# mli43/Cuda-Optimization-for-SpMM

Hardware: AMD Instinct MI355X
Metric: SpMM GFLOP/s, large_25605 (n4c6-b13) CSR x dense K=128 fp32 (higher is better)
Workload: dtype f32

## Files before the change

cuda-optimization-for-spmm_amd/csrc/row_gather.hpp:

```cpp
#pragma once
#include <algorithm>
#include <cstdio>
#include <cstdlib>
#include <type_traits>

#include "spmm_common.hpp"

namespace mispmm {

#ifdef MISPMM_STAMPS
static __device__ unsigned long long *mispmm_stamp_buf = nullptr;
constexpr uint32_t kStampLaunches = 32;
#endif

struct CsrRows {
    const uint32_t *rowPtrs;
    static constexpr bool kPadded = false;
    __device__ __forceinline__ void extent(uint32_t row, size_t &base, uint32_t &len) const {
        const uint32_t s = rowPtrs[row];
        base = s;
        len = rowPtrs[row + 1] - s;
    }
};

struct UniformRows {
    uint32_t width;
    static constexpr bool kPadded = false;
    __device__ __forceinline__ void extent(uint32_t row, size_t &base, uint32_t &len) const {
        base = static_cast<size_t>(row) * width;
        len = width;
    }
};

struct EllRows {
    uint32_t width;
    static constexpr bool kPadded = true;
    __device__ __forceinline__ void extent(uint32_t row, size_t &base, uint32_t &len) const {
        base = static_cast<size_t>(row) * width;
        len = width;
    }
};

struct SpanRows {
    const uint32_t *spans;
    static constexpr bool kPadded = false;
};

constexpr uint32_t kMaxBatch = 16;
struct BatchPtrs {
    const float *b[kMaxBatch];
    float *c[kMaxBatch];
};
template <bool BATCHED> struct BatchArg {};
template <> struct BatchArg<true> {
    BatchPtrs p;
};

template <int G, int VEC, class Acc, bool CBUF, class Rows, int BLOCK = 256, int UMAX = 16, bool ROLL = false, int SLOTS = 16,
          bool BATCHED = false, bool MAPPED = false>
#ifndef MISPMM_X_WAVES
#define MISPMM_X_WAVES 5
#endif
__device__ __forceinline__ void row_gather_body(const uint32_t bx, const uint32_t by, const uint32_t bz,
    uint32_t M, uint32_t rb_chunk, uint32_t tiling, uint32_t cols_per_part, uint32_t N, uint32_t ldb, Rows rows,
    const uint32_t *__restrict__ colIdxs, const float *__restrict__ vals, uint32_t b_bytes,
    const float *__restrict__ B_one, float *__restrict__ C_one, uint32_t c_bytes, uint32_t ldc,
    const uint32_t *__restrict__ rowMap, BatchArg<BATCHED> batch
#ifdef MISPMM_STAMPS
    , uint32_t stamp_launch
#endif
    ) {
#ifdef MISPMM_STAMPS
    unsigned long long stamp[5];
    stamp[0] = wall_clock64();
#endif
#ifdef MISPMM_X_PRIO
    __builtin_amdgcn_s_setprio(3);
#endif
    const float *__restrict__ B = B_one;
    float *__restrict__ C = C_one;
    if constexpr (BATCHED) {
        B = batch.p.b[bz];
        C = batch.p.c[bz];
    }
    constexpr int GROUPS = BLOCK / G;
    constexpr int U = G < UMAX ? G : UMAX;
    using vec_t = typename VecOf<VEC>::type;
    const uint32_t lane = threadIdx.x % G;
    const uint32_t xcd = bx & 7u, slot = bx >> 3;
    const uint32_t log2p = tiling & 0xFFu;
    const uint32_t p = xcd & ((1u << log2p) - 1u), q = xcd >> log2p;
    const uint32_t row = (p * rb_chunk + slot) * GROUPS + threadIdx.x / G;
    const bool row_ok = row < M;
    const uint32_t col0 = q * cols_per_part + by * (G * VEC) + lane * VEC;
    const bool col_ok = col0 < min(N, (q + 1) * cols_per_part);
    size_t row_base = 0;
    uint32_t row_len = 0;
    uint32_t ptr_lo = 0, ptr_hi = 0;
    uint32_t out_row = row;
    if constexpr (std::is_same_v<Rows, CsrRows>) {
        const uint32_t rr = min(row, M - 1u);
        ptr_lo = rows.rowPtrs[rr];
        ptr_hi = rows.rowPtrs[rr + 1];
    } else if constexpr (std::is_same_v<Rows, SpanRows>) {
        if (row_ok) {
            using u4 = uint32_t __attribute__((ext_vector_type(4)));
            const u4 span = *reinterpret_cast<const u4 *>(rows.spans + static_cast<size_t>(row) * 4u);
            out_row = span[0];
            row_base = span[1];
            row_len = span[2] - span[1];
        }
    } else {
        if (row_ok) rows.extent(row, row_base, row_len);
    }
    auto resolve_extent = [&] {
        if constexpr (std::is_same_v<Rows, CsrRows>) {
            row_base = ptr_lo;
            row_len = row_ok ? ptr_hi - ptr_lo : 0u;
        }
    };
    typename Acc::T acc[VEC];
#pragma unroll
    for (int v = 0; v < VEC; ++v) acc[v] = 0;
    auto load_out_row = [&] {
        if constexpr (MAPPED) {
            if (row_ok) out_row = rowMap[row];
        }
    };
    const rsrc_t rsrc = make_rsrc(B, b_bytes);
    const uint32_t lane_off = col_ok ? col0 * 4u : kDropLoad;
    const uint32_t ldb4 = ldb * 4u;

    auto fetch = [&](size_t mine, uint32_t &off, float &val) {
        const uint32_t col = colIdxs[mine];
        val = vals[mine];
        off = col * ldb4;
        if constexpr (Rows::kPadded) {
            if (col == 0xFFFFFFFFu) {
                off = kDropLoad;
                val = 0.f;
            }
        }
    };
    auto issue = [&](auto nb_tag, vec_t *bv, float *av, uint32_t my_off, float my_val, uint32_t j, uint32_t cnt) {
        constexpr int NB = decltype(nb_tag)::value;
#pragma unroll
        for (int u = 0; u < NB; ++u) {
            const uint32_t src = (j + u) & (G - 1);
            const uint32_t off = __shfl(my_off, src, G);
            const float a = __shfl(my_val, src, G);
            bool live = j + u < cnt;
            if constexpr (Rows::kPadded) live = live && off != kDropLoad;
            av[u] = live ? a : 0.f;
            bv[u] = buffer_load_vec<VEC>(rsrc, live ? off + lane_off : kDropLoad, 0);
        }
    };
    auto consume = [&](auto nb_tag, const vec_t *bv, const float *av) {
        constexpr int NB = decltype(nb_tag)::value;
#pragma unroll
        for (int u = 0; u < NB; ++u) {
#pragma unroll
            for (int v = 0; v < VEC; ++v) Acc::mac(acc[v], av[u], vec_get<VEC>(bv[u], v));
        }
    };
    using FullBatch = std::integral_constant<int, U>;

    if constexpr (ROLL && G <= 16) {
        constexpr int SC = SLOTS, E = (SC + G - 1) / G;
        static_assert(SLOTS == 16 || (SLOTS > U && SLOTS < 16) || (G == 16 && SLOTS == 32), "unsupported slot count");
        uint32_t nxt_off[E];
        float nxt_val[E];
        auto fetch_super = [&](uint32_t base) {
#pragma unroll
            for (int e = 0; e < E; ++e) {
                const uint32_t idx = base + e * G + lane;
                fetch(row_base + min(idx, row_len - 1), nxt_off[e], nxt_val[e]);
                if (idx >= row_len) {
                    nxt_off[e] = kDropLoad;
                    nxt_val[e] = 0.f;
                }
            }
        };
        if constexpr (std::is_same_v<Rows, CsrRows>) {
            const uint32_t guess = tiling >> 8;
            if (guess != 0) {
                row_base = static_cast<size_t>(row) * guess;
                row_len = row_ok ? guess : 0u;
                if (row_len != 0) fetch_super(0);
                const size_t bet_base = row_base;
                const uint32_t bet_len = row_len;
                resolve_extent();
                const bool hit = __all(!row_ok || (row_base == bet_base && row_len == bet_len));
                if (!hit && row_len != 0) fetch_super(0);
            } else {
                resolve_extent();
                if (row_len != 0) fetch_super(0);
            }
        } else {
            if (row_len != 0) fetch_super(0);
        }
        load_out_row();
#ifdef MISPMM_X_PRIO
        __builtin_amdgcn_s_setprio(0);
#endif
#ifdef MISPMM_STAMPS
        asm volatile("s_waitcnt vmcnt(0)" ::: "memory");
        stamp[1] = wall_clock64();
#endif
        for (uint32_t base = 0; base < row_len; base += SC) {
            uint32_t my_off[E];
            float my_val[E];
#pragma unroll
            for (int e = 0; e < E; ++e) {
                my_off[e] = nxt_off[e];
                my_val[e] = nxt_val[e];
            }
            if (base + SC < row_len) fetch_super(base + SC);
            vec_t bv[U];
            float av[U];
            auto issue_one = [&](auto slot_tag, vec_t &b, float &a) {
                constexpr int S = decltype(slot_tag)::value;
                const uint32_t off = group_bcast<G, S % G>(my_off[S / G]);
                const float c = __builtin_bit_cast(float, group_bcast<G, S % G>(__builtin_bit_cast(uint32_t, my_val[S / G])));
                a = c;
                b = buffer_load_vec<VEC, MISPMM_B_LOAD_AUX>(rsrc, off + lane_off, 0);
            };
            auto consume_one = [&](const vec_t &b, float a) {
                if constexpr (VEC == 4 && std::is_same_v<Acc, AccRefWide>) {
                    Acc::mac4(acc, a, vec_get<VEC>(b, 0), vec_get<VEC>(b, 1), vec_get<VEC>(b, 2), vec_get<VEC>(b, 3));
                } else {
#pragma unroll
                    for (int v = 0; v < VEC; ++v) Acc::mac(acc[v], a, vec_get<VEC>(b, v));
                }
            };
            auto live_from = [&](auto from_tag) {
                constexpr int FROM = decltype(from_tag)::value;
                bool live = false;
                static_for<0, E>([&](auto e_tag) {
                    constexpr int E0 = decltype(e_tag)::value * G;
                    if constexpr (E0 + G > FROM) {
                        const bool in_range = (E0 >= FROM) || (lane >= static_cast<uint32_t>(FROM > E0 ? FROM - E0 : 0));
                        live = live || (in_range && my_off[decltype(e_tag)::value] != kDropLoad);
                    }
                });
                return __any(live);
            };
            auto roll = [&](auto scx_tag) {
                constexpr int SCX = decltype(scx_tag)::value;
                static_for<0, U>([&](auto s) { issue_one(s, bv[decltype(s)::value], av[decltype(s)::value]); });
                __builtin_amdgcn_sched_barrier(0);
                static_for<0, SCX>([&](auto s) {
                    constexpr int S = decltype(s)::value;
                    consume_one(bv[S % U], av[S % U]);
                    if constexpr (S + U < SCX) {
                        if constexpr (VEC == 4) asm volatile("" : "+v"(acc[0]), "+v"(acc[1]), "+v"(acc[2]), "+v"(acc[3]) : : "memory");
                        else if constexpr (VEC == 2) asm volatile("" : "+v"(acc[0]), "+v"(acc[1]) : : "memory");
                        else asm volatile("" : "+v"(acc[0]) : : "memory");
                        __builtin_amdgcn_sched_barrier(0);
                        issue_one(std::integral_constant<int, S + U>{}, bv[S % U], av[S % U]);
                        __builtin_amdgcn_sched_barrier(0);
                    }
                });
            };
            if constexpr (Rows::kPadded) {
                if (!live_from(std::integral_constant<int, 0>{})) continue;
            }
            if (!live_from(std::integral_constant<int, U>{})) {
                static_for<0, U>([&](auto s) { issue_one(s, bv[decltype(s)::value], av[decltype(s)::value]); });
                __builtin_amdgcn_sched_barrier(0);
                static_for<0, U>([&](auto s) { consume_one(bv[decltype(s)::value], av[decltype(s)::value]); });
            } else if constexpr (SC == 16) {
#ifdef MISPMM_X_FEWBODIES
                if (!live_from(std::integral_constant<int, 14>{})) roll(std::integral_constant<int, 14>{});
                else roll(std::integral_constant<int, 16>{});
#else
                if (!live_from(std::integral_constant<int, 10>{})) roll(std::integral_constant<int, 10>{});
                else if (!live_from(std::integral_constant<int, 12>{})) roll(std::integral_constant<int, 12>{});
                else if (!live_from(std::integral_constant<int, 14>{})) roll(std::integral_constant<int, 14>{});
                else roll(std::integral_constant<int, 16>{});
#endif
            } else {
                roll(std::integral_constant<int, SC>{});
            }
        }
    } else if (resolve_extent(), !__any(row_len > static_cast<uint32_t>(U))) {
        load_out_row();
        if (row_len != 0) {
            uint32_t my_off;
            float my_val;
            fetch(row_base + min(lane, row_len - 1), my_off, my_val);
            vec_t bv[U];
            float av[U];
            issue(FullBatch{}, bv, av, my_off, my_val, 0, row_len);
            __builtin_amdgcn_sched_barrier(0);
            consume(FullBatch{}, bv, av);
        }
    } else {
        uint32_t nxt_off = 0;
        float nxt_val = 0.f;
        if (row_len != 0) fetch(row_base + min(lane, row_len - 1), nxt_off, nxt_val);
        load_out_row();
        for (uint32_t base = 0; base < row_len; base += G) {
            const uint32_t cnt = min(static_cast<uint32_t>(G), row_len - base);
            const uint32_t my_off = nxt_off;
            const float my_val = nxt_val;
            if (base + G < row_len) fetch(row_base + min(base + G + lane, row_len - 1), nxt_off, nxt_val);
            for (uint32_t j = 0; j < cnt; j += U) {
                vec_t bv[U];
                float av[U];
                issue(FullBatch{}, bv, av, my_off, my_val, j, cnt);
                __builtin_amdgcn_sched_barrier(0);
                consume(FullBatch{}, bv, av);
            }
        }
    }
#ifdef MISPMM_STAMPS
    if constexpr (VEC == 4) asm volatile("" : "+v"(acc[0]), "+v"(acc[1]), "+v"(acc[2]), "+v"(acc[3]) : : "memory");
    stamp[2] = wall_clock64();
#endif
    if (row_ok && col_ok) {
        vec_t out;
#pragma unroll
        for (int v = 0; v < VEC; ++v) vec_set<VEC>(out, v, Acc::finish(acc[v]));
        if constexpr (CBUF) {
            buffer_store_vec_c<VEC>(make_rsrc(C, c_bytes), (out_row * ldc + col0) * 4u, out);
        } else {
            store_vec<VEC>(C + static_cast<size_t>(out_row) * ldc + col0, out);
        }
    }
#ifdef MISPMM_STAMPS
    stamp[3] = wall_clock64();
    asm volatile("s_waitcnt vmcnt(0)" ::: "memory");
    stamp[4] = wall_clock64();
    if (mispmm_stamp_buf && (threadIdx.x & 63) == 0) {
        const uint32_t wpb = blockDim.x / 64;
        const size_t waves_per_launch = static_cast<size_t>(gridDim.x) * gridDim.y * wpb;
        unsigned long long *o = mispmm_stamp_buf + (stamp_launch * waves_per_launch +
            (static_cast<size_t>(by) * gridDim.x + bx) * wpb + (threadIdx.x >> 6)) * 8;
#pragma unroll
        for (int i = 0; i < 5; ++i) o[i] = stamp[i];
        o[5] = static_cast<unsigned long long>(__builtin_amdgcn_s_getreg((31 << 11) | 4));
        o[6] = static_cast<unsigned long long>(__builtin_amdgcn_s_getreg((31 << 11) | 20));
    }
#endif
}

template <int G, int VEC, class Acc, bool CBUF, class Rows, int BLOCK = 256, int UMAX = 16, bool ROLL = false, int SLOTS = 16,
          bool BATCHED = false, bool MAPPED = false>
__global__ __launch_bounds__(BLOCK, ROLL ? (UMAX > 8 ? 3 : MISPMM_X_WAVES) : 1) void row_gather_kernel(
    uint32_t M, uint32_t rb_chunk, uint32_t tiling, uint32_t cols_per_part, uint32_t N, uint32_t ldb, Rows rows,
    const uint32_t *__restrict__ colIdxs, const float *__restrict__ vals, uint32_t b_bytes,
    const float *__restrict__ B_one, float *__restrict__ C_one, uint32_t c_bytes, uint32_t ldc,
    const uint32_t *__restrict__ rowMap, BatchArg<BATCHED> batch
#ifdef MISPMM_STAMPS
    , uint32_t stamp_launch
#endif
    ) {
    row_gather_body<G, VEC, Acc, CBUF, Rows, BLOCK, UMAX, ROLL, SLOTS, BATCHED, MAPPED>(blockIdx.x, blockIdx.y, blockIdx.z, M, rb_chunk, tiling,
                                                                                    cols_per_part, N, ldb, rows, colIdxs, vals, b_bytes, B_one,
                                                                                    C_one, c_bytes, ldc, rowMap, batch
#ifdef MISPMM_STAMPS
                                                                                    , stamp_launch
#endif
    );
}

struct alignas(16) LineTail {
    float *C;
    uint32_t c_bytes, ldc4;
    const uint32_t *rowMap;
    uint64_t reserved;
};
struct LineBatchPair {
    const float *b;
    float *c;
};
template <bool BATCHED> struct LineBatch {};
template <> struct alignas(16) LineBatch<true> {
    LineBatchPair p[kMaxBatch];
};

template <int G, class Acc, bool PADDED, int SLOTS, bool BATCHED, bool MAPPED>
__global__ __launch_bounds__(128, MISPMM_X_WAVES) void row_line_kernel(
    const uint32_t *__restrict__ colIdxs, const float *__restrict__ vals, const float *__restrict__ B_one, uint32_t b_bytes,
    uint32_t ldb4, uint32_t width, uint32_t M, uint32_t rb_chunk, uint32_t log2p, uint32_t cols_per_part,
    LineTail tail, LineBatch<BATCHED> batch
#ifdef MISPMM_STAMPS
    , uint32_t stamp_launch
#endif
    ) {
#ifdef MISPMM_STAMPS
    unsigned long long stamp[5];
    stamp[0] = wall_clock64();
#endif
    constexpr int VEC = 4, BLOCK = 128, GROUPS = BLOCK / G, U = 8, E = (SLOTS + G - 1) / G;
    static_assert((G == 8 || G == 16) && SLOTS > U && SLOTS < 16, "rows of 9..14 slots");
    using vec_t = f32x4;
    const float *__restrict__ B = B_one;
    float *__restrict__ C = tail.C;
    const uint32_t c_bytes = tail.c_bytes, ldc4 = tail.ldc4;
    const uint32_t *__restrict__ rowMap = tail.rowMap;
    if constexpr (BATCHED) {
        const LineBatchPair pr = batch.p[blockIdx.z];
        B = pr.b;
        C = pr.c;
    }
    __builtin_amdgcn_sched_barrier(0);
    const uint32_t lane = threadIdx.x % G;
    const uint32_t xcd = blockIdx.x & 7u, slot = blockIdx.x >> 3;
    const uint32_t p = xcd & ((1u << log2p) - 1u), q = xcd >> log2p;
    const uint32_t row = (p * rb_chunk + slot) * GROUPS + threadIdx.x / G;
    const bool row_ok = row < M;
    const uint32_t part_col = blockIdx.y * (G * VEC) + lane * VEC;
    const bool col_ok = part_col < cols_per_part;
    const uint32_t col0 = q * cols_per_part + part_col;

    const uint32_t a_bytes = M * width * 4u;
    const rsrc_t colrs = make_rsrc(colIdxs, a_bytes), valrs = make_rsrc(vals, a_bytes);
    const uint32_t row_pos = row * width;
    uint32_t raw_col[E], raw_val[E];
#pragma unroll
    for (int e = 0; e < E; ++e) {
        const uint32_t idx = static_cast<uint32_t>(e * G) + lane;
        const uint32_t pos4 = row_ok ? (row_pos + min(idx, width - 1u)) * 4u : kDropLoad;
        raw_col[e] = __builtin_amdgcn_raw_buffer_load_b32(colrs, pos4, 0, 0);
        raw_val[e] = __builtin_amdgcn_raw_buffer_load_b32(valrs, pos4, 0, 0);
    }
    __builtin_amdgcn_sched_barrier(0);
    uint32_t out_row = row;
    if constexpr (MAPPED) out_row = __builtin_amdgcn_raw_buffer_load_b32(make_rsrc(rowMap, M * 4u), row_ok ? row * 4u : kDropLoad, 0, 0);
    const rsrc_t brs = make_rsrc(B, b_bytes);
    const rsrc_t crs = make_rsrc(C, c_bytes);
    const uint32_t lane_off = col_ok ? col0 * 4u : kDropLoad;
    const uint32_t store_col4 = col0 * 4u;
    const bool store_ok = row_ok && col_ok;
#ifdef MISPMM_STAMPS
    asm volatile("s_waitcnt vmcnt(0)" ::: "memory");
    stamp[1] = wall_clock64();
#endif
    uint32_t my_off[E], my_val[E];
#pragma unroll
    for (int e = 0; e < E; ++e) {
        const uint32_t idx = static_cast<uint32_t>(e * G) + lane;
        bool drop = !row_ok || idx >= width;
        if constexpr (PADDED) drop = drop || raw_col[e] == 0xFFFFFFFFu;
        const uint32_t keep = drop ? 0u : 0xFFFFFFFFu;
        my_off[e] = ((raw_col[e] * ldb4) & keep) | (drop ? kDropLoad : 0u);
        my_val[e] = raw_val[e] & keep;
    }
    typename Acc::T acc[VEC];
#pragma unroll
    for (int v = 0; v < VEC; ++v) acc[v] = 0;
    vec_t bv[U];
    float av[U];
    auto issue_one = [&](auto slot_tag, vec_t &b, float &a) {
        constexpr int S = decltype(slot_tag)::value;
        const uint32_t off = group_bcast<G, S % G>(my_off[S / G]);
        a = __builtin_bit_cast(float, group_bcast<G, S % G>(my_val[S / G]));
        b = buffer_load_vec<VEC, MISPMM_B_LOAD_AUX>(brs, off + lane_off, 0);
    };
    auto consume_one = [&](const vec_t &b, float a) {
        if constexpr (std::is_same_v<Acc, AccRefWide>) {
            Acc::mac4(acc, a, b[0], b[1], b[2], b[3]);
        } else {
#pragma unroll
            for (int v = 0; v < VEC; ++v) Acc::mac(acc[v], a, b[v]);
        }
    };
    static_for<0, U>([&](auto s) { issue_one(s, bv[decltype(s)::value], av[decltype(s)::value]); });
    __builtin_amdgcn_sched_barrier(0);
    static_for<0, SLOTS>([&](auto s) {
        constexpr int S = decltype(s)::value;
        consume_one(bv[S % U], av[S % U]);
        if constexpr (S + U < SLOTS) {
            asm volatile("" : "+v"(acc[0]), "+v"(acc[1]), "+v"(acc[2]), "+v"(acc[3]) : : "memory");
            __builtin_amdgcn_sched_barrier(0);
            issue_one(std::integral_constant<int, S + U>{}, bv[S % U], av[S % U]);
            __builtin_amdgcn_sched_barrier(0);
        }
    });
#ifdef MISPMM_STAMPS
    asm volatile("" : "+v"(acc[0]), "+v"(acc[1]), "+v"(acc[2]), "+v"(acc[3]) : : "memory");
    stamp[2] = wall_clock64();
#endif
    vec_t out;
#pragma unroll
    for (int v = 0; v < VEC; ++v) out[v] = Acc::finish(acc[v]);
    buffer_store_vec_c<VEC>(crs, store_ok ? out_row * ldc4 + store_col4 : kDropLoad, out);
#ifdef MISPMM_STAMPS
    stamp[3] = wall_clock64();
    asm volatile("s_waitcnt vmcnt(0)" ::: "memory");
    stamp[4] = wall_clock64();
    if (mispmm_stamp_buf && (threadIdx.x & 63) == 0) {
        const uint32_t wpb = blockDim.x / 64;
        const size_t waves_per_launch = static_cast<size_t>(gridDim.x) * gridDim.y * wpb;
        unsigned long long *o = mispmm_stamp_buf + (stamp_launch * waves_per_launch +
            (static_cast<size_t>(blockIdx.y) * gridDim.x + blockIdx.x) * wpb + (threadIdx.x >> 6)) * 8;
#pragma unroll
        for (int i = 0; i < 5; ++i) o[i] = stamp[i];
        o[5] = static_cast<unsigned long long>(__builtin_amdgcn_s_getreg((31 << 11) | 4));
        o[6] = static_cast<unsigned long long>(__builtin_amdgcn_s_getreg((31 << 11) | 20));
    }
#endif
}

template <class Rows> constexpr const char *rows_tag() {
    if constexpr (std::is_same_v<Rows, CsrRows>) return "csr";
    else if constexpr (std::is_same_v<Rows, UniformRows>) return "uniform";
    else if constexpr (std::is_same_v<Rows, SpanRows>) return "spans";
    else return "ell";
}

struct RowGatherArgs {
    hipStream_t stream;
    uint32_t M, K;
    const uint32_t *colIdxs;
    const float *vals, *B;
    uint32_t N, ldb;
    float *C;
    uint32_t ldc;
    uint32_t mean_row_len = 0;
    const uint32_t *rowMap = nullptr;
    uint32_t row_len_guess = 0;
    uint32_t batch = 0;
    const float *const *B_list = nullptr;
    float *const *C_list = nullptr;
};

inline bool &row_gather_declined() {
    static thread_local bool declined = false;
    return declined;
}

inline uint32_t uniform_guess(uint32_t M, uint64_t nnz) {
    return (M != 0 && nnz != 0 && nnz % M == 0) ? static_cast<uint32_t>(nnz / M) : 0u;
}

struct XcdTiling {
    uint32_t log2p, q;
    bool sc1;
};

inline XcdTiling xcd_tiling(uint32_t N, int vec, uint32_t K) {
    struct Env {
        int log2p = -1;
        uint32_t q = 0;
        int sc1 = -1;
        Env() {
            if (const char *e = knob_str("MISPMM_CSR_TILING")) {
                unsigned pp = 8, qq = 1;
                if (sscanf(e, "%u,%u", &pp, &qq) == 2 && pp * qq == 8 && (pp == 1 || pp == 2 || pp == 4 || pp == 8)) {
                    log2p = pp == 1 ? 0 : pp == 2 ? 1 : pp == 4 ? 2 : 3;
                    q = qq;
                }
            }
            if (const char *e = knob_str("MISPMM_STORE_SC1")) sc1 = e[0] != '0';
        }
    };
    static const Env env;
    XcdTiling t{3u, 1u, true};
    if (vec >= 2 && N >= 128 && N % 64 == 0) {
        uint32_t q = 2;
        while (q < 8 && N / (q * 2) >= 64 && N % (q * 2 * 32) == 0) q *= 2;
        if (q == 4 && N == 256 && static_cast<uint64_t>(K) * 256u > (4ull << 20)) q = 8;
        t.q = q;
        t.log2p = q == 2 ? 2u : q == 4 ? 1u : 0u;
    }
    if (env.log2p >= 0) {
        t.log2p = static_cast<uint32_t>(env.log2p);
        t.q = env.q;
    }
    while (t.q > 1 && (N % t.q != 0 || (N / t.q) % (8u * vec) != 0)) {
        t.q >>= 1;
        ++t.log2p;
    }
    if (env.sc1 >= 0) t.sc1 = env.sc1 != 0;
    return t;
}

template <int G, int VEC, class Acc, class Rows, int BLOCK, int UMAX = 16, bool ROLL = false, int SLOTS = 16>
void launch_row_gather_b(const RowGatherArgs &a, const Rows &rows, const XcdTiling &t) {
    const uint32_t cols_per_part = a.N / t.q;
    const uint32_t rb = ceil_div(a.M, BLOCK / G);
    const uint32_t rb_chunk = ceil_div(rb, 1u << t.log2p);
    dim3 grid(8u * rb_chunk, ceil_div(cols_per_part, G * VEC));
    const uint32_t b_bytes = static_cast<uint32_t>(static_cast<uint64_t>(a.K) * a.ldb * 4u);
    const uint64_t c_bytes = static_cast<uint64_t>(a.M) * a.ldc * 4u;
    static const bool guess_on = knob_int("MISPMM_ROW_GUESS", 1) != 0;
    const uint32_t tiling = t.log2p | ((std::is_same_v<Rows, CsrRows> && ROLL && guess_on && a.row_len_guess < (1u << 24)) ? a.row_len_guess << 8 : 0u);
    note_kernel("row_gather<G%d,V%d,%s,%s,B%d,U%d,%s,S%d> xcd %ux%u%s%s", G, VEC, acc_tag<Acc>(), rows_tag<Rows>(), BLOCK, UMAX,
                ROLL ? "roll" : "batch", SLOTS, 1u << t.log2p, t.q, a.batch ? " batched" : "", a.rowMap ? " plan-order" : "");
#ifdef MISPMM_STAMPS
    static uint32_t stamp_counter = 0;
    const uint32_t stamp_launch = stamp_counter++ % kStampLaunches;
#define MISPMM_STAMP_ARG , stamp_launch
#else
#define MISPMM_STAMP_ARG
#endif
    if constexpr (ROLL && BLOCK == 128 && UMAX == 8 && G <= 16) {
        if (a.batch > 0) {
            BatchArg<true> arg;
            for (uint32_t i = 0; i < kMaxBatch; ++i) {
                arg.p.b[i] = a.B_list[i < a.batch ? i : 0];
                arg.p.c[i] = a.C_list[i < a.batch ? i : 0];
            }
            grid.z = a.batch;
            if (a.rowMap)
                hipLaunchKernelGGL((row_gather_kernel<G, VEC, Acc, true, Rows, BLOCK, UMAX, ROLL, SLOTS, true, true>), grid, dim3(BLOCK), 0, a.stream,
                                   a.M, rb_chunk, tiling, cols_per_part, a.N, a.ldb, rows, a.colIdxs, a.vals, b_bytes, nullptr, nullptr,
                                   static_cast<uint32_t>(c_bytes), a.ldc, a.rowMap, arg MISPMM_STAMP_ARG);
            else
                hipLaunchKernelGGL((row_gather_kernel<G, VEC, Acc, true, Rows, BLOCK, UMAX, ROLL, SLOTS, true>), grid, dim3(BLOCK), 0, a.stream,
                                   a.M, rb_chunk, tiling, cols_per_part, a.N, a.ldb, rows, a.colIdxs, a.vals, b_bytes, nullptr, nullptr,
                                   static_cast<uint32_t>(c_bytes), a.ldc, nullptr, arg MISPMM_STAMP_ARG);
            return;
        }
    }
    if (a.batch > 0) {
        for (uint32_t i = 0; i < a.batch; ++i) {
            RowGatherArgs one = a;
            one.batch = 0;
            one.B = a.B_list[i];
            one.C = a.C_list[i];
            launch_row_gather_b<G, VEC, Acc, Rows, BLOCK, UMAX, ROLL, SLOTS>(one, rows, t);
        }
        return;
    }
    if constexpr (ROLL && BLOCK == 128 && UMAX == 8 && G <= 16 && VEC == 4) {
        if (a.rowMap) {
            hipLaunchKernelGGL((row_gather_kernel<G, VEC, Acc, true, Rows, BLOCK, UMAX, ROLL, SLOTS, false, true>), grid, dim3(BLOCK), 0, a.stream,
                               a.M, rb_chunk, tiling, cols_per_part, a.N, a.ldb, rows, a.colIdxs, a.vals, b_bytes, a.B, a.C,
                               static_cast<uint32_t>(c_bytes), a.ldc, a.rowMap, BatchArg<false>{} MISPMM_STAMP_ARG);
            return;
        }
    }
    if (a.rowMap) {
        row_gather_declined() = true;
        return;
    }
    if (t.sc1 && c_bytes <= 0x7FFFFFFFull)
        hipLaunchKernelGGL((row_gather_kernel<G, VEC, Acc, true, Rows, BLOCK, UMAX, ROLL, SLOTS>), grid, dim3(BLOCK), 0, a.stream, a.M, rb_chunk,
                           tiling, cols_per_part, a.N, a.ldb, rows, a.colIdxs, a.vals, b_bytes, a.B, a.C,
                           static_cast<uint32_t>(c_bytes), a.ldc, a.rowMap, BatchArg<false>{} MISPMM_STAMP_ARG);
    else
        hipLaunchKernelGGL((row_gather_kernel<G, VEC, Acc, false, Rows, BLOCK, UMAX, ROLL, SLOTS>), grid, dim3(BLOCK), 0, a.stream, a.M, rb_chunk,
                           tiling, cols_per_part, a.N, a.ldb, rows, a.colIdxs, a.vals, b_bytes, a.B, a.C, 0u, a.ldc, a.rowMap, BatchArg<false>{} MISPMM_STAMP_ARG);
#undef MISPMM_STAMP_ARG
}

inline bool row_line_fits(uint32_t M, uint32_t width, uint32_t ldc) {
    return static_cast<uint64_t>(M) * width * 4u <= 0x7FFFFFFFull && static_cast<uint64_t>(M) * ldc * 4u <= 0x7FFFFFFFull;
}

template <int G, class Acc, class Rows, int SLOTS>
bool launch_row_line(const RowGatherArgs &a, const Rows &rows, const XcdTiling &t) {
    static const bool line_on = knob_int("MISPMM_LINE", 1) != 0;
    if (!line_on || !t.sc1 || !row_line_fits(a.M, rows.width, a.ldc)) return false;
    constexpr int VEC = 4, BLOCK = 128;
    const uint32_t cols_per_part = a.N / t.q;
    const uint32_t rb_chunk = ceil_div(ceil_div(a.M, BLOCK / G), 1u << t.log2p);
    dim3 grid(8u * rb_chunk, ceil_div(cols_per_part, G * VEC));
    const uint32_t b_bytes = static_cast<uint32_t>(static_cast<uint64_t>(a.K) * a.ldb * 4u);
    LineTail tail{a.C, static_cast<uint32_t>(static_cast<uint64_t>(a.M) * a.ldc * 4u), a.ldc * 4u, a.rowMap, 0};
    note_kernel("row_gather<G%d,V%d,%s,%s,B%d,U%d,%s,S%d> xcd %ux%u%s%s", G, VEC, acc_tag<Acc>(), rows_tag<Rows>(), BLOCK, 8, "line", SLOTS,
                1u << t.log2p, t.q, a.batch ? " batched" : "", a.rowMap ? " plan-order" : "");
#ifdef MISPMM_STAMPS
    static uint32_t stamp_counter = 0;
    const uint32_t stamp_launch = stamp_counter++ % kStampLaunches;
#define MISPMM_STAMP_ARG , stamp_launch
#else
#define MISPMM_STAMP_ARG
#endif
#define MISPMM_LINE_LAUNCH(BATCHED, MAPPED, B_PTR, BATCH_ARG)                                                                          \
    hipLaunchKernelGGL((row_line_kernel<G, Acc, Rows::kPadded, SLOTS, BATCHED, MAPPED>), grid, dim3(BLOCK), 0, a.stream, a.colIdxs, a.vals, \
                       B_PTR, b_bytes, a.ldb * 4u, rows.width, a.M, rb_chunk, t.log2p, cols_per_part, tail, BATCH_ARG MISPMM_STAMP_ARG)
    if (a.batch > 0) {
        LineBatch<true> arg;
        for (uint32_t i = 0; i < kMaxBatch; ++i) arg.p[i] = LineBatchPair{a.B_list[i < a.batch ? i : 0], a.C_list[i < a.batch ? i : 0]};
        tail.C = nullptr;
        grid.z = a.batch;
        if (a.rowMap) MISPMM_LINE_LAUNCH(true, true, nullptr, arg);
        else MISPMM_LINE_LAUNCH(true, false, nullptr, arg);
    } else if (a.rowMap) {
        MISPMM_LINE_LAUNCH(false, true, a.B, LineBatch<false>{});
    } else {
        MISPMM_LINE_LAUNCH(false, false, a.B, LineBatch<false>{});
    }
#undef MISPMM_LINE_LAUNCH
#undef MISPMM_STAMP_ARG
    return true;
}

template <int G, int VEC, class Acc, class Rows>
void launch_row_gather(const RowGatherArgs &a, const Rows &rows, const XcdTiling &t) {
    static const int block = knob_int("MISPMM_BLOCK", 128);
    static const int umax = knob_int("MISPMM_UMAX", 8);
    static const int roll = knob_int("MISPMM_ROLL", 1);
    if constexpr ((G == 16 || G == 8) && VEC == 4 && (std::is_same_v<Rows, UniformRows> || std::is_same_v<Rows, EllRows>)) {
        static const bool slots = knob_int("MISPMM_SLOTS", 1) != 0;
        if (roll && slots) {
            if (rows.width > 8 && rows.width <= 10) {
                if (launch_row_line<G, Acc, Rows, 10>(a, rows, t)) return;
                return launch_row_gather_b<G, VEC, Acc, Rows, 128, 8, true, 10>(a, rows, t);
            }
            if (rows.width > 10 && rows.width <= 12) {
                if (launch_row_line<G, Acc, Rows, 12>(a, rows, t)) return;
                return launch_row_gather_b<G, VEC, Acc, Rows, 128, 8, true, 12>(a, rows, t);
            }
#ifdef MISPMM_TUNING
            if constexpr (G == 16 && std::is_same_v<Rows, UniformRows>) {
                if (rows.width > 12 && rows.width <= 14 && block == 64) return launch_row_gather_b<G, VEC, Acc, Rows, 64, 8, true, 14>(a, rows, t);
                if (rows.width > 12 && rows.width <= 14 && block == 256) return launch_row_gather_b<G, VEC, Acc, Rows, 256, 8, true, 14>(a, rows, t);
            }
#endif
            if (rows.width > 12 && rows.width <= 14) {
                if (launch_row_line<G, Acc, Rows, 14>(a, rows, t)) return;
                return launch_row_gather_b<G, VEC, Acc, Rows, 128, 8, true, 14>(a, rows, t);
            }
        }
    }
    if constexpr (G == 16 && VEC == 4 && std::is_same_v<Rows, CsrRows>) {
        static const int deep_env = knob_int("MISPMM_DEEP", -1);
        const bool deep = deep_env >= 0 ? deep_env != 0 : a.mean_row_len >= 24;
        if (roll && deep) return launch_row_gather_b<G, VEC, Acc, Rows, 128, 16, true, 32>(a, rows, t);
    }
    if constexpr (G <= 16) {
        if (roll) return launch_row_gather_b<G, VEC, Acc, Rows, 128, 8, true>(a, rows, t);
    }
    if (block == 64) launch_row_gather_b<G, VEC, Acc, Rows, 64, 8>(a, rows, t);
    else if (block == 256) launch_row_gather_b<G, VEC, Acc, Rows, 256, 8>(a, rows, t);
    else if (umax == 16) launch_row_gather_b<G, VEC, Acc, Rows, 128, 16>(a, rows, t);
    else launch_row_gather_b<G, VEC, Acc, Rows, 128, 8>(a, rows, t);
}

inline bool row_gather_supports_map(uint32_t M, uint32_t K, uint32_t N, uint32_t ldc, int vec, uint32_t mean_row_len) {
    if (vec != 4 || static_cast<uint64_t>(M) * ldc * 4u > 0x7FFFFFFFull || mean_row_len >= 24) return false;
    if (knob_int("MISPMM_ROLL", 1) == 0 || knob_int("MISPMM_BLOCK", 128) != 128 || knob_int("MISPMM_UMAX", 8) != 8 ||
        knob_int("MISPMM_GROUP", 0) > 16 || knob_int("MISPMM_DEEP", -1) == 1)
        return false;
    const XcdTiling t = xcd_tiling(N, vec, K);
    return t.sc1 && (N / t.q) % 32 == 0;
}

template <class Acc, class Rows>
void launch_row_gather_auto(const RowGatherArgs &a, const Rows &rows, int vec) {
    const XcdTiling t = xcd_tiling(a.N, vec, a.K);
    static const int group_env = knob_int("MISPMM_GROUP", 0);
    const uint32_t cpp = a.N / t.q;
    const int g = group_env ? group_env
                  : (vec == 4 && cpp % 64 == 0) ? 16
                  : (vec == 4 && cpp % 32 == 0) ? 8
                                                : pick_group(cpp, vec);
    try_const<4, 2, 1>(vec, [&](auto v) {
        try_const<8, 16, 32, 64>(g, [&](auto gg) { launch_row_gather<decltype(gg)::value, decltype(v)::value, Acc, Rows>(a, rows, t); });
    });
}

}
```

Baseline: 6781.

## Walk batched operands in one block with a register ring prefetching the next B

Behind a compile-time flag, the batched line kernel keeps each block resident across several batch entries instead of launching one z-slice per operand. Column offsets and coefficients are broadcast once and reused, and a ring of B-vector registers issues loads for the next operand while the current one is being accumulated. The intent is to cut per-block setup and hide load latency across operands. In exchange it adds register pressure and serialises batch entries within a block, which lowers parallelism when grid.z shrinks.

After: 6575. -3.1%, worse.

```diff
diff --git a/cuda-optimization-for-spmm_amd/csrc/row_gather.hpp b/cuda-optimization-for-spmm_amd/csrc/row_gather.hpp
--- a/cuda-optimization-for-spmm_amd/csrc/row_gather.hpp
+++ b/cuda-optimization-for-spmm_amd/csrc/row_gather.hpp
@@ -378,7 +378,18 @@
 template <bool BATCHED> struct LineBatch {};
 template <> struct alignas(16) LineBatch<true> {
     LineBatchPair p[kMaxBatch];
-};
+#ifdef MISPMM_X_BATCH_WALK
+    uint32_t count;
+#endif
+};
+
+#ifdef MISPMM_X_BATCH_WALK
+#ifdef MISPMM_X_LINE_RING
+constexpr int line_batch_ring(int slots) { return slots == 14 ? MISPMM_X_LINE_RING : slots; }
+#else
+constexpr int line_batch_ring(int slots) { return slots == 14 ? 7 : slots; }
+#endif
+#endif
 
 template <int G, class Acc, bool PADDED, int SLOTS, bool BATCHED, bool MAPPED>
 __global__ __launch_bounds__(128, MISPMM_X_WAVES) void row_line_kernel(
@@ -448,6 +459,65 @@
         my_off[e] = ((raw_col[e] * ldb4) & keep) | (drop ? kDropLoad : 0u);
         my_val[e] = raw_val[e] & keep;
     }
+#ifdef MISPMM_X_BATCH_WALK
+    if constexpr (BATCHED) {
+        constexpr int R = line_batch_ring(SLOTS);
+        static_assert(SLOTS % R == 0 && R <= SLOTS, "a slot keeps its ring register from operand to operand");
+        uint32_t voff[SLOTS];
+        float coef[SLOTS];
+        static_for<0, SLOTS>([&](auto s) {
+            constexpr int S = decltype(s)::value;
+            voff[S] = group_bcast<G, S % G>(my_off[S / G]) + lane_off;
+            coef[S] = __builtin_bit_cast(float, group_bcast<G, S % G>(my_val[S / G]));
+        });
+        const uint32_t count = batch.count, zstep = gridDim.z;
+        uint32_t z = blockIdx.z;
+        rsrc_t cur_b = brs, cur_c = crs;
+        vec_t ring[R];
+        static_for<0, R>([&](auto s) { ring[decltype(s)::value] = buffer_load_vec<VEC, MISPMM_B_LOAD_AUX>(cur_b, voff[decltype(s)::value], 0); });
+        __builtin_amdgcn_sched_barrier(0);
+        const uint32_t store_off = store_ok ? out_row * ldc4 + store_col4 : kDropLoad;
+        auto walk_one = [&](auto roll_on, const rsrc_t &next_b) {
+            typename Acc::T acc[VEC];
+#pragma unroll
+            for (int v = 0; v < VEC; ++v) acc[v] = 0;
+            static_for<0, SLOTS>([&](auto s) {
+                constexpr int S = decltype(s)::value;
+                const vec_t b = ring[S % R];
+                if constexpr (std::is_same_v<Acc, AccRefWide>) {
+                    Acc::mac4(acc, coef[S], b[0], b[1], b[2], b[3]);
+                } else {
+#pragma unroll
+                    for (int v = 0; v < VEC; ++v) Acc::mac(acc[v], coef[S], b[v]);
+                }
+                if constexpr (S + R < SLOTS || decltype(roll_on)::value) {
+                    asm volatile("" : "+v"(acc[0]), "+v"(acc[1]), "+v"(acc[2]), "+v"(acc[3]) : : "memory");
+                    __builtin_amdgcn_sched_barrier(0);
+                    if constexpr (S + R < SLOTS) ring[S % R] = buffer_load_vec<VEC, MISPMM_B_LOAD_AUX>(cur_b, voff[S + R], 0);
+                    else ring[S % R] = buffer_load_vec<VEC, MISPMM_B_LOAD_AUX>(next_b, voff[S + R - SLOTS], 0);
+                    __builtin_amdgcn_sched_barrier(0);
+                }
+            });
+            vec_t out;
+#pragma unroll
+            for (int v = 0; v < VEC; ++v) out[v] = Acc::finish(acc[v]);
+            buffer_store_vec_c<VEC>(cur_c, store_off, out);
+        };
+        LineBatchPair nxt = batch.p[min(z + zstep, kMaxBatch - 1u)];
+        while (z + zstep < count) {
+            const LineBatchPair after = batch.p[min(z + 2u * zstep, kMaxBatch - 1u)];
+            __builtin_amdgcn_sched_barrier(0);
+            const rsrc_t next_b = make_rsrc(nxt.b, b_bytes);
+            walk_one(std::true_type{}, next_b);
+            cur_b = next_b;
+            cur_c = make_rsrc(nxt.c, c_bytes);
+            nxt = after;
+            z += zstep;
+        }
+        walk_one(std::false_type{}, cur_b);
+        return;
+    }
+#endif
     typename Acc::T acc[VEC];
 #pragma unroll
     for (int v = 0; v < VEC; ++v) acc[v] = 0;
@@ -652,6 +722,13 @@
     return static_cast<uint64_t>(M) * width * 4u <= 0x7FFFFFFFull && static_cast<uint64_t>(M) * ldc * 4u <= 0x7FFFFFFFull;
 }
 
+#ifdef MISPMM_X_BATCH_WALK
+inline uint32_t line_batch_grid_z(uint32_t batch) {
+    static const int walk_env = knob_int("MISPMM_BATCH_WALK", 1);
+    return walk_env > 0 ? std::min(static_cast<uint32_t>(walk_env), batch) : batch;
+}
+#endif
+
 template <int G, class Acc, class Rows, int SLOTS>
 bool launch_row_line(const RowGatherArgs &a, const Rows &rows, const XcdTiling &t) {
     static const bool line_on = knob_int("MISPMM_LINE", 1) != 0;
@@ -679,6 +756,10 @@
         for (uint32_t i = 0; i < kMaxBatch; ++i) arg.p[i] = LineBatchPair{a.B_list[i < a.batch ? i : 0], a.C_list[i < a.batch ? i : 0]};
         tail.C = nullptr;
         grid.z = a.batch;
+#ifdef MISPMM_X_BATCH_WALK
+        arg.count = a.batch;
+        grid.z = line_batch_grid_z(a.batch);
+#endif
         if (a.rowMap) MISPMM_LINE_LAUNCH(true, true, nullptr, arg);
         else MISPMM_LINE_LAUNCH(true, false, nullptr, arg);
     } else if (a.rowMap) {
```
